# seiya-kumada/3d_gaussian_splatting

Measured on AMD Instinct MI355X. Metric: forward+backward iters/s at 1080p, 1M Gaussians; PSNR vs CPU ref, higher is better.
Workload: dtype f32; 1 GPU; 1m_1080p: 1000000 Gaussians, 1920x1080, SH degree 3, fwd+bwd; gaussians=1000000, width=1920, height=1080, sh_degree=3, parallelism=single GPU

## Files before the change

### 3d_gaussian_splatting_amd/csrc/gsr_blend.hip

```cpp
#include "gsr_kernels.h"

namespace gsr {
namespace {

constexpr int kPPL = 4;

__device__ inline int xcd_tile(int b, int nwg) {
    const int q = nwg / 8, r = nwg % 8;
    const int xcd = b % 8, local = b / 8;
    return (xcd < r ? xcd * (q + 1) : r * (q + 1) + (xcd - r) * q) + local;
}

template <int CTRL>
__device__ inline float dpp_f(float x) {
    return __int_as_float(__builtin_amdgcn_update_dpp(0, __float_as_int(x), CTRL, 0xF, 0xF, false));
}

template <int N>
__device__ __forceinline__ void quad_reduce(float (&v)[N]) {
#pragma unroll
    for (int i = 0; i < N; ++i) v[i] += dpp_f<0xB1>(v[i]);
#pragma unroll
    for (int i = 0; i < N; ++i) v[i] += dpp_f<0x4E>(v[i]);
#pragma unroll
    for (int i = 0; i < N; ++i) asm volatile("" : "+v"(v[i]));
}



struct BlendGeom {
    int W, H, grid_x, ty0, nwg;
    int vgy, vh;
    uint32_t ck_slots;
    int ck_fixed;
    float bg0, bg1, bg2;
    uint32_t cap;
};

__device__ __forceinline__ float edge_min_q(float a, float b, float c, float k, float u, float v0, float v1) {
    const float vs = fminf(fmaxf(k * u, v0), v1);
    return fmaf(fmaf(c, vs, b * u), vs, a * u * u);
}

__device__ inline uint32_t stripe_mask(const float4 r0, const float4 r1, const float4 r2, float bx0, float by0) {
    const float ex = r2.y, ey = r2.z;
    if (!(ex >= 0.0f) || r0.x + ex < bx0 || r0.x - ex > bx0 + 15.0f) return 0u;
    const float ylo = r0.y - ey, yhi = r0.y + ey;
    const float A = -r0.z, B = -r0.w, C = -r1.x;
    const bool pd = A > 0.0f && C > 0.0f && 4.0f * A * C - B * B > 0.0f;
    const float bound = fmaf(fmaxf(r2.w + 7.99435343f, 0.0f), 1.02f, 0.05f);
    const float x0 = bx0 - r0.x, x1 = bx0 + 15.0f - r0.x;
    const float kc = -B * __builtin_amdgcn_rcpf(2.0f * C), ka = -B * __builtin_amdgcn_rcpf(2.0f * A);
    uint32_t m = 0;
#pragma unroll
    for (int p = 0; p < kPPL; ++p) {
        const float s0 = by0 + 4.0f * p;
        bool hit = yhi >= s0 && ylo <= s0 + 3.0f;
        if (hit && pd) {
            const float y0 = s0 - r0.y, y1 = s0 + 3.0f - r0.y;
            const bool inside = x0 <= 0.0f && x1 >= 0.0f && y0 <= 0.0f && y1 >= 0.0f;
            const float q = fminf(fminf(edge_min_q(A, B, C, kc, x0, y0, y1), edge_min_q(A, B, C, kc, x1, y0, y1)),
                                  fminf(edge_min_q(C, B, A, ka, y0, x0, x1), edge_min_q(C, B, A, ka, y1, x0, x1)));
            hit = inside || q <= bound;
        }
        m |= hit ? (1u << p) : 0u;
    }
    return m;
}

__device__ __forceinline__ float pair_alpha(float e, float L, float& oG) {
    oG = __builtin_amdgcn_exp2f(e);
    const float a = __builtin_amdgcn_fmed3f(oG, 0.0f, 0.99f);
    return (e <= L && oG >= (1.0f / 255.0f)) ? a : 0.0f;
}

__device__ __forceinline__ float pair_alpha_keep(float e, float L, float& oG, bool& keep) {
    oG = __builtin_amdgcn_exp2f(e);
    keep = e <= L && oG >= (1.0f / 255.0f);
    return keep ? __builtin_amdgcn_fmed3f(oG, 0.0f, 0.99f) : 0.0f;
}


constexpr int kF6Batch4 = 256;
constexpr int kF6Wpe = 8;
template <class T>
__device__ __forceinline__ T aux_arg() { return T{}; }
template <class T>
__device__ __forceinline__ T aux_arg(const T& a) { return a; }
__device__ __forceinline__ float aux_value(uint32_t key, int inv) {
    const float z = __uint_as_float(key);
    return inv ? 1.0f / z : z;
}
constexpr int kF6AuxWpe = 7;
template <int NW, class... AX>
__global__ __launch_bounds__(64 * NW) __attribute__((amdgpu_waves_per_eu(NW == 2 ? (sizeof...(AX) ? kF6AuxWpe : kF6Wpe) : 1))) void blend_forward_kernel(const BlendGeom geo,
                                                                const uint2* __restrict__ ranges,
                                                                const uint32_t* __restrict__ sorted_gid,
                                                                const float4* __restrict__ rec,
                                                                float* __restrict__ out_color,
                                                                float* __restrict__ final_T,
                                                                float* __restrict__ accum,
                                                                uint32_t* __restrict__ term,
                                                                float4* __restrict__ ck,
                                                                uint8_t* __restrict__ mk, const AX... axp) {
    constexpr bool AUX = sizeof...(AX) > 0;
    static_assert(sizeof...(AX) <= 1, "one aux argument");
    const F6Aux ax = aux_arg<F6Aux>(axp...);
    constexpr int PPL = kPPL / NW;
    constexpr int BATCH = NW > 2 ? kF6Batch4 : 64 * NW;
    static_assert(BATCH % 64 == 0 && BATCH <= 64 * NW, "F6 batch");
    constexpr int kCW = NW > 2 ? kBandChunkWork : kChunkWork;
    __shared__ float4 srec[BATCH * 3];
    __shared__ uint32_t smk[BATCH];
    __shared__ uint32_t slive[NW];
    __shared__ float svz[AUX ? BATCH : 1];
    const int tl = xcd_tile(blockIdx.x, geo.nwg);
    const int tile = tl + geo.ty0 * geo.grid_x;
    const int tx = tile % geo.grid_x, ty = tile / geo.grid_x;
    const int tid = threadIdx.x, w = tid >> 6, lane = tid & 63;
    const int px = tx * kTile + (lane & 15);
    const float pfx = (float)px;
    const int view = ty / geo.vgy, tyl = ty - view * geo.vgy;
    const float bx0 = (float)(tx * kTile), by0 = (float)(tyl * kTile);
    float pfy[PPL], T[PPL], C0[PPL], C1[PPL], C2[PPL];
    float Z[PPL];
#pragma unroll
    for (int p = 0; p < PPL; ++p) {
        const int pyl = tyl * kTile + (lane >> 4) + 4 * (w * PPL + p);
        pfy[p] = (float)pyl;
        T[p] = (px < geo.W && pyl < geo.vh) ? 1.0f : -1.0f;
        C0[p] = C1[p] = C2[p] = 0.0f;
        Z[p] = 0.0f;
    }
    const uint2 range = ranges[tile];
    const int n = (int)(range.y - range.x);
    float vref = 0.0f;
    if constexpr (AUX) {
        if (n > 0) vref = aux_value(ax.depth_key[sorted_gid[range.x]], ax.inv);
    }
    uint32_t* const table = term + (size_t)tl * kMaxChunks;
    int nck = 0;
    int work = 0;
    int tend = n;
    uint8_t* const ckm = reinterpret_cast<uint8_t*>(ck + (size_t)geo.ck_slots * 256);
    auto checkpoint = [&](size_t slot, uint32_t lv) {
        float4* dst = ck + (size_t)slot * 256;
#pragma unroll
        for (int p = 0; p < PPL; ++p) {
            const bool on = (lv >> p) & 1u;
            if (on) dst[64 * (w * PPL + p) + lane] = make_float4(T[p], C0[p], C1[p], C2[p]);
            if constexpr (AUX) {
                if (on) ax.ckz[(size_t)slot * 256 + 64 * (w * PPL + p) + lane] = Z[p];
            }
            if (lane == 0) ckm[4 * (size_t)slot + w * PPL + p] = on ? 1 : 0;
        }
    };
    int quota = kCW;
    auto merge_chunks = [&]() {
        constexpr int kKeep = (kMaxChunks - 1) / 2;
        float4* const ckt = ck + ck_slot_of(geo.ck_fixed, range.x, tl, 1) * 256 - 256;
        uint8_t* const ckmt = ckm + (ck_slot_of(geo.ck_fixed, range.x, tl, 1) - 1) * 4;
#pragma unroll 1
        for (int k = 1; k <= kKeep; ++k) {
#pragma unroll 1
            for (int p = 0; p < PPL; ++p) {
                const int i = 64 * (w * PPL + p) + lane;
                ckt[256 * k + i] = ckt[512 * k + i];
                if constexpr (AUX) {
                    float* const ckzt = ax.ckz + ck_slot_of(geo.ck_fixed, range.x, tl, 1) * 256 - 256;
                    ckzt[256 * k + i] = ckzt[512 * k + i];
                }
                if (lane == 0) ckmt[4 * k + w * PPL + p] = ckmt[8 * k + w * PPL + p];
            }
            if (tid == 0) table[k] = table[2 * k];
        }
        nck = kKeep;
        work += quota;
        quota *= 2;
    };
    uint32_t g_next = tid < BATCH && tid < n ? sorted_gid[range.x + tid] : 0u;
    for (int base = 0; base < n; base += BATCH) {
        uint32_t live = 0;
#pragma unroll
        for (int p = 0; p < PPL; ++p) live |= __any(T[p] > 0.0f) ? (1u << p) : 0u;
        if (lane == 0) slive[w] = live << (w * PPL);
        if (tid < BATCH && base + tid < n) {
            const uint32_t g = g_next;
            if (base + BATCH + tid < n) g_next = sorted_gid[range.x + base + BATCH + tid];
            const float4* r = rec + 3 * (size_t)g;
            const float4 r0 = r[0], r1 = r[1], r2 = r[2];
            srec[3 * tid + 0] = r0;
            srec[3 * tid + 1] = r1;
            srec[3 * tid + 2] = r2;
            smk[tid] = stripe_mask(r0, r1, r2, bx0, by0);
            if constexpr (AUX) svz[tid] = aux_value(ax.depth_key[g], ax.inv) - vref;
            mk[range.x + base + tid] = (uint8_t)smk[tid];
        } else if (tid < BATCH) {
            smk[tid] = 0u;
        }
        __syncthreads();
        uint32_t tile_live = 0;
#pragma unroll
        for (int i = 0; i < NW; ++i) tile_live |= slive[i];
        if (tile_live == 0) {
            tend = base;
            break;
        }
        const int cnt = (n - base) < BATCH ? (n - base) : BATCH;
        int visited = 0;
        for (int c0 = 0; c0 < cnt; c0 += 64) {
            const uint32_t sm = smk[c0 + lane];
            if (__builtin_expect(work >= quota && nck == kMaxChunks - 1, 0)) merge_chunks();
            if (work >= quota && nck < kMaxChunks - 1) {
                ++nck;
                checkpoint(ck_slot_of(geo.ck_fixed, range.x, tl, nck), live);
                if (tid == 0) table[nck] = (uint32_t)(base + c0);
                work = 0;
            }
            const uint32_t tm = sm & tile_live;
            work += __popcll(__ballot(tm & 1u)) + __popcll(__ballot(tm & 2u)) + __popcll(__ballot(tm & 4u)) +
                    __popcll(__ballot(tm & 8u));
            if (!live) continue;
            const uint32_t mine = (sm >> (w * PPL)) & ((1u << PPL) - 1u);
            uint64_t todo = __ballot((mine & live) != 0u && c0 + lane < cnt);
            if constexpr (PPL == 1) {
                while (todo) {
                    const int ka = c0 + __builtin_ctzll(todo);
                    todo &= todo - 1;
                    const bool two = todo != 0;
                    const int kb = two ? c0 + __builtin_ctzll(todo) : ka;
                    if (two) todo &= todo - 1;
                    const float4 a0 = srec[3 * ka + 0], a1 = srec[3 * ka + 1], a2 = srec[3 * ka + 2];
                    const float4 b0 = srec[3 * kb + 0], b1 = srec[3 * kb + 1], b2 = srec[3 * kb + 2];
                    const float dxa = a0.x - pfx, dxb = b0.x - pfx;
                    const float dya = a0.y - pfy[0], dyb = b0.y - pfy[0];
                    const float ea = fmaf(fmaf(a1.x, dya, a0.w * dxa), dya, fmaf(a0.z * dxa, dxa, a2.w));
                    const float eb = fmaf(fmaf(b1.x, dyb, b0.w * dxb), dyb, fmaf(b0.z * dxb, dxb, b2.w));
                    float oGa, oGb;
                    const float aa = pair_alpha(ea, a2.w, oGa);
                    const float ab = pair_alpha(eb, b2.w, oGb);
                    {
                        const float w = aa * T[0];
                        const float tT = T[0] - w;
                        const bool ok = tT >= 0.0001f;
                        const float wgt = ok ? w : 0.0f;
                        C0[0] = fmaf(a1.z, wgt, C0[0]);
                        C1[0] = fmaf(a1.w, wgt, C1[0]);
                        C2[0] = fmaf(a2.x, wgt, C2[0]);
                        if constexpr (AUX) Z[0] = fmaf(svz[ka], wgt, Z[0]);
                        T[0] = ok ? tT : -fabsf(T[0]);
                    }
                    if (two) {
                        const float w = ab * T[0];
                        const float tT = T[0] - w;
                        const bool ok = tT >= 0.0001f;
                        const float wgt = ok ? w : 0.0f;
                        C0[0] = fmaf(b1.z, wgt, C0[0]);
                        C1[0] = fmaf(b1.w, wgt, C1[0]);
                        C2[0] = fmaf(b2.x, wgt, C2[0]);
                        if constexpr (AUX) Z[0] = fmaf(svz[kb], wgt, Z[0]);
                        T[0] = ok ? tT : -fabsf(T[0]);
                    }
                    const int before = visited;
                    visited += two ? 2 : 1;
                    if ((before >> 3) != (visited >> 3)) {
                        live = __any(T[0] > 0.0f) ? 1u : 0u;
                        if (live == 0) break;
                    }
                }
                continue;
            }
            while (todo) {
                const int kk = __builtin_ctzll(todo);
                todo &= todo - 1;
                const int k = c0 + kk;
                const float4 r0 = srec[3 * k + 0];
                const float4 r1 = srec[3 * k + 1];
                const float4 r2 = srec[3 * k + 2];
                const float dx = r0.x - pfx;
                const float bdx = r0.w * dx;
                const float K = fmaf(r0.z * dx, dx, r2.w);
                float vz = 0.0f;
                if constexpr (AUX) vz = svz[k];
#pragma unroll
                for (int p = 0; p < PPL; ++p) {
                    const float dy = r0.y - pfy[p];
                    const float e = fmaf(fmaf(r1.x, dy, bdx), dy, K);
                    float oG;
                    const float a = pair_alpha(e, r2.w, oG);
                    const float w = a * T[p];
                    const float tT = T[p] - w;
                    const bool ok = tT >= 0.0001f;
                    const float wgt = ok ? w : 0.0f;
                    C0[p] = fmaf(r1.z, wgt, C0[p]);
                    C1[p] = fmaf(r1.w, wgt, C1[p]);
                    C2[p] = fmaf(r2.x, wgt, C2[p]);
                    if constexpr (AUX) Z[p] = fmaf(vz, wgt, Z[p]);
                    T[p] = ok ? tT : -fabsf(T[p]);
                }
                if ((++visited & 7) == 0) {
                    uint32_t lv = 0;
#pragma unroll
                    for (int p = 0; p < PPL; ++p) lv |= __any(T[p] > 0.0f) ? (1u << p) : 0u;
                    live = lv;
                    if (live == 0) break;
                }
            }
        }
        __syncthreads();
    }
    if (tid == 0) {
        table[0] = (uint32_t)tend;
        for (int c = nck + 1; c < kMaxChunks; ++c) table[c] = 0xFFFFFFFFu;
    }
    const size_t npix = (size_t)geo.W * geo.vh;
    float* const oc = out_color + (size_t)view * 3 * npix;
    float* const ac = accum + (size_t)view * 3 * npix;
    float* const fT = final_T + (size_t)view * npix;
#pragma unroll
    for (int p = 0; p < PPL; ++p) {
        const int pyl = tyl * kTile + (lane >> 4) + 4 * (w * PPL + p);
        if (px < geo.W && pyl < geo.vh) {
            const size_t pix = (size_t)pyl * geo.W + px;
            const float Tf = fabsf(T[p]);
            fT[pix] = Tf;
            ac[pix] = C0[p];
            ac[npix + pix] = C1[p];
            ac[2 * npix + pix] = C2[p];
            oc[pix] = C0[p] + Tf * geo.bg0;
            oc[npix + pix] = C1[p] + Tf * geo.bg1;
            oc[2 * npix + pix] = C2[p] + Tf * geo.bg2;
            if constexpr (AUX) {
                ax.accum_z[pix] = Z[p];
                ax.out_depth[pix] = fmaf(vref, 1.0f - Tf, Z[p]);
                ax.out_alpha[pix] = 1.0f - Tf;
            }
        }
    }
}

constexpr int kPark = 4;
constexpr int kParkSlot = 16 * 12 + 8;
static_assert(kParkSlot % 32 == 8 && kParkSlot % 4 == 0, "flush banks / float4 alignment");
template <bool AUX = false>
__device__ __forceinline__ void park_flush(const float* qpark, const uint32_t* sjl, uint32_t kpack, int parked,
                                           float* p8f, float* p1, uint8_t* fl, int lane, float* pz = nullptr) {
    __syncthreads();
    const int slot = lane & 3, c = lane >> 2;
    if (c < (AUX ? 10 : 9) && slot < parked) {
        const float* q = qpark + slot * kParkSlot + c;
        float t[4] = {-0.f, -0.f, -0.f, -0.f};
#pragma unroll
        for (int i = 0; i < 16; ++i) t[i & 3] += q[i * 12];
        const uint32_t j = sjl[(kpack >> (6 * slot)) & 63u];
        if (j != 0xFFFFFFFFu) {
            float* dst = c < 8 ? p8f + 8 * (size_t)j + c : p1 + j;
            if constexpr (AUX) dst = c == 9 ? pz + j : dst;
            *dst = (t[0] + t[1]) + (t[2] + t[3]);
            if (c == 8) fl[j] = 1;
        }
    }
    __syncthreads();
}

constexpr int kB1AuxWpe = 5;
template <bool PF = false, class... AX>
__global__ __launch_bounds__(64) __attribute__((amdgpu_waves_per_eu(PF ? 4 : (sizeof...(AX) ? kB1AuxWpe : 6)))) void blend_backward_kernel(const BlendGeom geo,
                                                            const uint2* __restrict__ ranges,
                                                            const uint32_t* __restrict__ sorted_gid,
                                                            const uint4* __restrict__ rect,
                                                            const float4* __restrict__ rec,
                                                            const float* __restrict__ final_T,
                                                            const float* __restrict__ accum,
                                                            const float* __restrict__ dL_dpix,
                                                            float* __restrict__ p8f,
                                                            float* __restrict__ p1,
                                                            uint8_t* __restrict__ fl,
                                                            const uint32_t* __restrict__ term,
                                                            const float4* __restrict__ ck,
                                                            const uint8_t* __restrict__ mk, const AX... axp) {
    constexpr bool AUX = sizeof...(AX) > 0;
    static_assert(sizeof...(AX) <= 1, "one aux argument");
    constexpr int SPW = kPPL;
    const B1Aux ax = aux_arg<B1Aux>(axp...);
    __shared__ float svz[AUX ? 64 : 1];
    __shared__ struct {
        float4 srec[64 * 3];
        uint32_t sjl[64];
        float qpark[kPark * kParkSlot];
        uint32_t sidx[64];
        uint32_t smv[64];
        uint32_t sgd[64];
    } lds;
    float4* const srec = lds.srec;
    uint32_t* const sjl = lds.sjl;
    float* const qpark = lds.qpark;
    const int lane = threadIdx.x;
    float* const qlane = qpark + (lane >> 2) * 12;
    int tl, chunk;
    {
        const int q = geo.nwg / 8, r = geo.nwg % 8, xcd = blockIdx.x % 8, local = (int)(blockIdx.x / 8);
        const int t0 = xcd < r ? xcd * (q + 1) : r * (q + 1) + (xcd - r) * q, nt = q + (xcd < r ? 1 : 0);
        const int per = q + 1;
        chunk = local / per;
        const int i = local - chunk * per;
        if (i >= nt) return;
        tl = t0 + i;
    }
    const int tile = tl + geo.ty0 * geo.grid_x;
    const uint2 range = ranges[tile];
    const int n_all = (int)(range.y - range.x);
    const uint32_t* table = term + (size_t)tl * kMaxChunks;
    const uint32_t tend = table[0];
    const uint32_t start_u = chunk == 0 ? 0u : table[chunk];
    if (start_u >= (uint32_t)n_all || start_u >= tend) return;
    const int start = (int)start_u;
    float vref = 0.0f;
    if constexpr (AUX) vref = aux_value(ax.depth_key[sorted_gid[range.x]], ax.inv);
    const uint32_t next = chunk + 1 < kMaxChunks ? table[chunk + 1] : 0xFFFFFFFFu;
    const int n = next < (uint32_t)n_all ? (int)next : n_all;
    const int tx = tile % geo.grid_x, ty = tile / geo.grid_x;
    const int col = lane >> 2, row = lane & 3;
    const int px = tx * kTile + col;
    const float pfx = (float)px;
    const int view = ty / geo.vgy, tyl = ty - view * geo.vgy;
    const size_t npix = (size_t)geo.W * geo.vh;
    final_T += (size_t)view * npix;
    accum += (size_t)view * 3 * npix;
    dL_dpix += (size_t)view * 3 * npix;
    float pfy[SPW], T[SPW], R[SPW], dp0[SPW], dp1[SPW], dp2[SPW];
    float dpz[SPW], v0[SPW], azS[SPW], azT[SPW], azA[SPW];
#pragma unroll
    for (int p = 0; p < SPW; ++p) {
        const int pyl = tyl * kTile + row + 4 * p;
        pfy[p] = (float)pyl;
        const bool in = px < geo.W && pyl < geo.vh;
        const size_t pix = in ? (size_t)pyl * geo.W + px : 0;
        const float Tfin = in ? final_T[pix] : 1.0f;
        dp0[p] = in ? dL_dpix[pix] : 0.0f;
        dp1[p] = in ? dL_dpix[npix + pix] : 0.0f;
        dp2[p] = in ? dL_dpix[2 * npix + pix] : 0.0f;
        const float sdp = in ? accum[pix] * dp0[p] + accum[npix + pix] * dp1[p] + accum[2 * npix + pix] * dp2[p]
                             : 0.0f;
        R[p] = sdp + Tfin * (geo.bg0 * dp0[p] + geo.bg1 * dp1[p] + geo.bg2 * dp2[p]);
        dpz[p] = 0.0f;
        if constexpr (AUX) {
            dpz[p] = in && ax.dL_ddepth ? ax.dL_ddepth[pix] : 0.0f;
            azA[p] = in && ax.dL_dalpha ? ax.dL_dalpha[pix] : 0.0f;
            azS[p] = in ? ax.accum_z[pix] : 0.0f;
            azT[p] = Tfin;
            const float atot = 1.0f - Tfin;
            v0[p] = atot > 1e-6f ? azS[p] / atot : 0.0f;
        } else {
            v0[p] = azS[p] = azT[p] = azA[p] = 0.0f;
        }
        T[p] = in ? 1.0f : -1.0f;
    }
    if (chunk > 0) {
        const size_t slot = ck_slot_of(geo.ck_fixed, range.x, tl, chunk);
        const float4* src = ck + slot * 256;
        const uint32_t on = *reinterpret_cast<const uint32_t*>(
            reinterpret_cast<const uint8_t*>(ck + (size_t)geo.ck_slots * 256) + 4 * slot);
#pragma unroll
        for (int p = 0; p < SPW; ++p) {
            if ((on >> (8 * p)) & 0xFFu) {
                const float4 c4 = src[64 * p + col + 16 * row];
                T[p] = c4.x;
                R[p] -= fmaf(c4.y, dp0[p], fmaf(c4.z, dp1[p], c4.w * dp2[p]));
                if constexpr (AUX) azS[p] -= ax.ckz[slot * 256 + 64 * p + col + 16 * row];
            } else {
                T[p] = -1.0f;
            }
        }
    }
    if constexpr (AUX) {
#pragma unroll
        for (int p = 0; p < SPW; ++p) {
            const float Tst = chunk > 0 ? fabsf(T[p]) : 1.0f;
            const float rem = azS[p] - v0[p] * (Tst - azT[p]);
            R[p] = R[p] + ((rem - (v0[p] + vref) * azT[p]) * dpz[p] - azT[p] * azA[p]);
        }
    }
    const int n_lim = n < (int)tend ? n : (int)tend;
    for (int base = start; base < n_lim;) {
        uint32_t live = 0;
#pragma unroll
        for (int p = 0; p < SPW; ++p) live |= __any(T[p] > 0.0f) ? (1u << p) : 0u;
        if (live == 0) break;
        static_assert(kB1Win == 4, "one mask word and four gids per lane");
        const uint32_t a0 = (range.x + (uint32_t)base) & ~(uint32_t)(kB1Win - 1);
        const uint32_t wd = *reinterpret_cast<const uint32_t*>(mk + a0 + 4 * lane);
        const uint4 gw = *reinterpret_cast<const uint4*>(sorted_gid + a0 + 4 * lane);
        const uint32_t gwa[4] = {gw.x, gw.y, gw.z, gw.w};
        uint32_t vis = 0;
#pragma unroll
        for (int i = 0; i < kB1Win; ++i) {
            const int e = (int)(a0 + kB1Win * lane + i - range.x);
            const uint32_t m = (wd >> (8 * i)) & 0xFu;
            if (e >= base && e < n_lim && (m & live)) vis |= 1u << i;
        }
        const uint32_t c = (uint32_t)__popc(vis);
        uint32_t incl = c;
#pragma unroll
        for (int o = 1; o < 64; o <<= 1) {
            const uint32_t y = __shfl_up(incl, o, 64);
            if (lane >= o) incl += y;
        }
        const uint32_t excl = incl - c;
        const uint32_t total = (uint32_t)__shfl(incl, 63, 64);
        const int cnt = total < 64u ? (int)total : 64;
        uint32_t pos = excl;
#pragma unroll
        for (int i = 0; i < kB1Win; ++i) {
            if ((vis >> i) & 1u) {
                if (pos < 64u) {
                    lds.sidx[pos] = a0 + kB1Win * lane + i - range.x;
                    lds.smv[pos] = (wd >> (8 * i)) & 0xFu;
                    lds.sgd[pos] = gwa[i];
                }
                ++pos;
            }
        }
        __syncthreads();
        base = total > 64u ? (int)lds.sidx[63] + 1 : (int)(a0 + 64 * kB1Win - range.x);
        if (cnt == 0) {
            __syncthreads();
            continue;
        }
        uint32_t jl = 0, smask = 0;
        if (lane < cnt) {
            const uint32_t g = lds.sgd[lane];
            const uint4 rr = rect[g];
            const int minx = rr.x & 0xFFFF, miny = rr.x >> 16, maxx = rr.y & 0xFFFF;
            const int y0 = miny > geo.ty0 ? miny : geo.ty0;
            jl = rr.z + (uint32_t)((ty - y0) * (maxx - minx) + (tx - minx));
            if (jl >= geo.cap) jl = 0xFFFFFFFFu;
            const float4* r = rec + 3 * (size_t)g;
            srec[3 * lane + 0] = r[0];
            srec[3 * lane + 1] = r[1];
            srec[3 * lane + 2] = r[2];
            if constexpr (AUX) svz[lane] = aux_value(ax.depth_key[g], ax.inv) - vref;
            smask = lds.smv[lane];
        }
        sjl[lane] = jl;
        __syncthreads();
        uint64_t todo = __ballot(lane < cnt);
        int visited = 0, parked = 0;
        uint32_t kpack = 0;
        auto record = [&](const int k, const float4 r0, const float4 r1, const float4 r2, const float vz) -> bool {
            const uint32_t m = (uint32_t)__builtin_amdgcn_readlane((int)smask, k) & live;
            const float dx = r0.x - pfx;
            const float bdx = r0.w * dx;
            const float K = fmaf(r0.z * dx, dx, r2.w);
            float s0 = -0.f, sy = -0.f, syy = -0.f, g0 = -0.f, g1 = -0.f, g2 = -0.f;
            float gz = -0.f;
            bool any = false;
            auto contribute = [&](const int p, const float a, const float w, const float oG, const float dy) {
                any = true;
                const float one_m = 1.0f - a;
                float cdp = fmaf(r1.z, dp0[p], fmaf(r1.w, dp1[p], r2.x * dp2[p]));
                if constexpr (AUX) {
                    cdp = fmaf(vz - v0[p], dpz[p], cdp);
                    gz = fmaf(w, dpz[p], gz);
                }
                R[p] = fmaf(-w, cdp, R[p]);
                const float dLda = fmaf(T[p], cdp, -R[p] * __builtin_amdgcn_rcpf(one_m));
                g0 = fmaf(w, dp0[p], g0);
                g1 = fmaf(w, dp1[p], g1);
                g2 = fmaf(w, dp2[p], g2);
                const float sv = oG * dLda;
                s0 += sv;
                const float svy = sv * dy;
                sy += svy;
                syy = fmaf(svy, dy, syy);
            };
#pragma unroll
            for (int p = 0; p < SPW; ++p) {
                if (!(m & (1u << p))) continue;
                const float dy = r0.y - pfy[p];
                const float e = fmaf(fmaf(r1.x, dy, bdx), dy, K);
                float oG;
                bool keep;
                const float a = pair_alpha_keep(e, r2.w, oG, keep);
                const float w = a * T[p];
                const float tT = T[p] - w;
                const bool ok = tT >= 0.0001f;
                if (ok && keep) contribute(p, a, w, oG, dy);
                T[p] = ok ? tT : -fabsf(T[p]);
            }
            if (__any(any)) {
                float u[AUX ? 7 : 6] = {s0, sy, syy, g0, g1, g2};
                if constexpr (AUX) u[6] = gz;
                quad_reduce(u);
                const float sx = u[0] * dx;
                float v[9] = {sx, u[1], sx * dx, u[1] * dx, u[2], u[0], u[3], u[4], u[5]};
                if ((lane & 3) == 0) {
                    float* dst = qlane + parked * kParkSlot;
                    *reinterpret_cast<float4*>(dst) = make_float4(v[0], v[1], v[2], v[3]);
                    *reinterpret_cast<float4*>(dst + 4) = make_float4(v[4], v[5], v[6], v[7]);
                    dst[8] = v[8];
                    if constexpr (AUX) dst[9] = u[6];
                }
                kpack |= (uint32_t)k << (6 * parked);
                if (++parked == kPark) {
                    park_flush<AUX>(qpark, sjl, kpack, parked, p8f, p1, fl, lane, ax.pz);
                    parked = 0;
                    kpack = 0;
                }
            }
            if ((++visited & 7) == 0) {
                uint32_t lv = 0;
#pragma unroll
                for (int p = 0; p < SPW; ++p) lv |= __any(T[p] > 0.0f) ? (1u << p) : 0u;
                live = lv;
                if (live == 0) return true;
            }
            return false;
        };
        if constexpr (PF) {
            if (todo) {
                int ka = __builtin_ctzll(todo);
                todo &= todo - 1;
                float4 a0 = srec[3 * ka + 0], a1 = srec[3 * ka + 1], a2 = srec[3 * ka + 2];
                float4 b0, b1, b2;
                float za = 0.0f, zb = 0.0f;
                if constexpr (AUX) za = svz[ka];
                while (true) {
                    const int kb = todo ? __builtin_ctzll(todo) : -1;
                    if (kb >= 0) {
                        todo &= todo - 1;
                        b0 = srec[3 * kb + 0];
                        b1 = srec[3 * kb + 1];
                        b2 = srec[3 * kb + 2];
                        if constexpr (AUX) zb = svz[kb];
                    }
                    if (record(ka, a0, a1, a2, za) || kb < 0) break;
                    ka = todo ? __builtin_ctzll(todo) : -1;
                    if (ka >= 0) {
                        todo &= todo - 1;
                        a0 = srec[3 * ka + 0];
                        a1 = srec[3 * ka + 1];
                        a2 = srec[3 * ka + 2];
                        if constexpr (AUX) za = svz[ka];
                    }
                    if (record(kb, b0, b1, b2, zb) || ka < 0) break;
                }
            }
        } else {
            while (todo) {
                const int k = __builtin_ctzll(todo);
                todo &= todo - 1;
                float vz = 0.0f;
                if constexpr (AUX) vz = svz[k];
                if (record(k, srec[3 * k + 0], srec[3 * k + 1], srec[3 * k + 2], vz)) break;
            }
        }
        if (parked) park_flush<AUX>(qpark, sjl, kpack, parked, p8f, p1, fl, lane, ax.pz);
        __syncthreads();
    }
}
}

constexpr int kF6FullWaves = 2, kF6BandWaves = 4, kF6BandTiles = 4096;

static BlendGeom make_geo(const gsr_camera& cam, const float bg[3], int ty0, int ty1, long long cap, int vgy, int vh) {
    BlendGeom g;
    g.W = cam.width;
    g.H = cam.height;
    g.vgy = vgy > 0 ? vgy : div_up(cam.height, kTile);
    g.vh = vgy > 0 ? vh : cam.height;
    g.grid_x = div_up(cam.width, kTile);
    g.ty0 = ty0;
    g.nwg = (ty1 - ty0) * g.grid_x;
    const long long full_tiles = (long long)div_up(cam.height, kTile) * g.grid_x;
    g.ck_slots = (uint32_t)ck_pool_slots(cap, full_tiles);
    g.ck_fixed = ck_fixed_layout(cap, full_tiles) ? 1 : 0;
    g.bg0 = bg[0];
    g.bg1 = bg[1];
    g.bg2 = bg[2];
    g.cap = cap > 0 ? (uint32_t)cap : 0u;
    return g;
}

static long long image_tiles(const BlendGeom& geo, int vgy) {
    return vgy > 0 ? (long long)geo.vgy * geo.grid_x : geo.nwg;
}
static bool aux_ok(const void* aux, const gsr_camera& cam, int ty0, int ty1, int vgy) {
    return !aux || (vgy <= 0 && ty0 == 0 && ty1 == div_up(cam.height, kTile));
}

int launch_blend_forward(const gsr_camera& cam, const float bg[3], int ty0, int ty1,
                         const uint2* ranges, const uint32_t* sorted_gid, const float4* rec,
                         float* out_color, float* final_T, float* accum, uint32_t* term, float4* ck, long long cap,
                         hipStream_t s, int vgy, int vh, uint8_t* mk, const F6Aux* aux) {
    if (!aux_ok(aux, cam, ty0, ty1, vgy)) return (int)hipErrorInvalidValue;
    const BlendGeom geo = make_geo(cam, bg, ty0, ty1, cap, vgy, vh);
    if (geo.nwg <= 0) return 0;
    auto launch = [&](auto nw, auto... ax) {
        constexpr int NW = decltype(nw)::value;
        hipLaunchKernelGGL((blend_forward_kernel<NW, decltype(ax)...>), dim3(geo.nwg), dim3(64 * NW), 0, s, geo, ranges,
                           sorted_gid, rec, out_color, final_T, accum, term, ck, mk, ax...);
    };
    auto pick = [&](auto... ax) {
        if (image_tiles(geo, vgy) >= kF6BandTiles)
            launch(std::integral_constant<int, kF6FullWaves>{}, ax...);
        else
            launch(std::integral_constant<int, kF6BandWaves>{}, ax...);
    };
    aux ? pick(*aux) : pick();
    return (int)hipGetLastError();
}

int launch_blend_backward(const gsr_camera& cam, const float bg[3], int ty0, int ty1,
                          const uint2* ranges, const uint32_t* sorted_gid, const uint4* rect,
                          const float4* rec, const float* final_T,
                          const float* accum, const float* dL_dpix, float* partial, long long cap,
                          const uint32_t* term, const float4* ck, hipStream_t s, int vgy, int vh,
                          const uint8_t* mk, const B1Aux* aux) {
    if (!aux_ok(aux, cam, ty0, ty1, vgy)) return (int)hipErrorInvalidValue;
    const BlendGeom geo = make_geo(cam, bg, ty0, ty1, cap, vgy, vh);
    if (geo.nwg <= 0) return 0;
    const PartLayout pl(cap, aux != nullptr);
    const int blocks = 8 * (geo.nwg / 8 + 1) * kMaxChunks;
    auto launch = [&](auto pf, auto... ax) {
        hipLaunchKernelGGL((blend_backward_kernel<decltype(pf)::value, decltype(ax)...>), dim3(blocks), dim3(64), 0, s,
                           geo, ranges, sorted_gid, rect, rec, final_T, accum, dL_dpix, at<float>(partial, pl.p8),
                           at<float>(partial, pl.p1), at<uint8_t>(partial, pl.fl), term, ck, mk, ax...);
    };
    auto pick = [&](auto... ax) {
        if (image_tiles(geo, vgy) < kF6BandTiles)
            launch(std::true_type{}, ax...);
        else
            launch(std::false_type{}, ax...);
    };
    B1Aux ax = aux ? *aux : B1Aux{};
    ax.pz = at<float>(partial, pl.pz);
    aux ? pick(ax) : pick();
    return (int)hipGetLastError();
}

int launch_clear_flags(float* partial, long long cap, bool aux, hipStream_t s) {
    if (cap <= 0) return 0;
    return (int)hipMemsetAsync(at<uint8_t>(partial, PartLayout(cap, aux).fl), 0, (size_t)cap, s);
}

}
```

Measured before the change: 923.7 iters/s.

## Compact staged Gaussian records in LDS and make park flushes bank-conflict-free

```diff
diff --git a/3d_gaussian_splatting_amd/csrc/gsr_blend.hip b/3d_gaussian_splatting_amd/csrc/gsr_blend.hip
--- a/3d_gaussian_splatting_amd/csrc/gsr_blend.hip
+++ b/3d_gaussian_splatting_amd/csrc/gsr_blend.hip
@@ -319,7 +319,7 @@
     float* const fT = final_T + (size_t)view * npix;
 #pragma unroll
     for (int p = 0; p < PPL; ++p) {
-        const int pyl = tyl * kTile + (lane >> 4) + 4 * (w * PPL + p);
+        const int pyl = (int)pfy[p];
         if (px < geo.W && pyl < geo.vh) {
             const size_t pix = (size_t)pyl * geo.W + px;
             const float Tf = fabsf(T[p]);
@@ -339,25 +339,76 @@
     }
 }
 
+constexpr int kStagedRec = 10;
+struct StagedRec {
+    float4 r0;
+    float4 h;
+    float L;
+};
+__device__ __forceinline__ StagedRec staged(const float2* srec, int k) {
+    const float2* p = srec + k * (kStagedRec / 2);
+    const float2 a = p[0], b = p[1], c = p[2], d = p[3];
+    return {make_float4(a.x, a.y, b.x, b.y), make_float4(c.x, c.y, d.x, d.y), p[4].x};
+}
+
 constexpr int kPark = 4;
-constexpr int kParkSlot = 16 * 12 + 8;
-static_assert(kParkSlot % 32 == 8 && kParkSlot % 4 == 0, "flush banks / float4 alignment");
+constexpr int kParkSlot = 16 * 12 + (kPark <= 4 ? 8 : 12);
+static_assert(kPark <= 5 && kParkSlot % 4 == 0, "flush banks / float4 alignment of the leaders' stores");
+struct FlushMap {
+    uint8_t sc[64];
+    bool ok;
+};
+constexpr FlushMap make_flush_map(int moments) {
+    FlushMap m{};
+    for (int l = 0; l < 64; ++l) m.sc[l] = 0xFF;
+    m.ok = true;
+    bool used[2][32] = {};
+    int fill[2] = {0, 0};
+    for (int s = 0; s < kPark; ++s)
+        for (int c = 0; c < moments; ++c) {
+            const int bank = (s * kParkSlot + c) % 32;
+            const int g = used[0][bank] ? 1 : 0;
+            if (used[g][bank] || fill[g] == 32) {
+                m.ok = false;
+                continue;
+            }
+            used[g][bank] = true;
+            m.sc[32 * g + fill[g]++] = (uint8_t)(s << 4 | c);
+        }
+    return m;
+}
+__device__ constexpr FlushMap kFlushMap = make_flush_map(9), kFlushMapAux = make_flush_map(10);
+static_assert(kFlushMap.ok && kFlushMapAux.ok, "flush lanes of one group on one LDS bank");
+static_assert(6 * kPark <= 32, "kpack");
+typedef const __attribute__((address_space(3))) float* LdsFloats;
+struct FlushLane {
+    LdsFloats q;
+    char* base;
+    uint32_t step;
+    int slot;
+    bool flag;
+};
 template <bool AUX = false>
-__device__ __forceinline__ void park_flush(const float* qpark, const uint32_t* sjl, uint32_t kpack, int parked,
-                                           float* p8f, float* p1, uint8_t* fl, int lane, float* pz = nullptr) {
+__device__ __forceinline__ FlushLane flush_lane(int lane, const float* qpark, float* p8f, float* p1, float* pz) {
+    const int sc = AUX ? kFlushMapAux.sc[lane] : kFlushMap.sc[lane];
+    const int c = sc & 15, slot = sc == 0xFF ? kPark : sc >> 4;
+    float* b = c < 8 ? p8f + c : p1;
+    if constexpr (AUX) b = c == 9 ? pz : b;
+    LdsFloats q = (LdsFloats)(qpark + (sc == 0xFF ? 0 : slot * kParkSlot + c));
+    asm volatile("" : "+v"(q));
+    return {q, reinterpret_cast<char*>(b), c < 8 ? 32u : 4u, slot, c == 8};
+}
+__device__ __forceinline__ void park_flush(const FlushLane f, const float2* srec, uint32_t kpack, int parked,
+                                           uint8_t* fl) {
     __syncthreads();
-    const int slot = lane & 3, c = lane >> 2;
-    if (c < (AUX ? 10 : 9) && slot < parked) {
-        const float* q = qpark + slot * kParkSlot + c;
+    if (f.slot < parked) {
         float t[4] = {-0.f, -0.f, -0.f, -0.f};
 #pragma unroll
-        for (int i = 0; i < 16; ++i) t[i & 3] += q[i * 12];
-        const uint32_t j = sjl[(kpack >> (6 * slot)) & 63u];
+        for (int i = 0; i < 16; ++i) t[i & 3] += f.q[i * 12];
+        const uint32_t j = __float_as_uint(srec[((kpack >> (6 * f.slot)) & 63u) * (kStagedRec / 2) + 4].y);
         if (j != 0xFFFFFFFFu) {
-            float* dst = c < 8 ? p8f + 8 * (size_t)j + c : p1 + j;
-            if constexpr (AUX) dst = c == 9 ? pz + j : dst;
-            *dst = (t[0] + t[1]) + (t[2] + t[3]);
-            if (c == 8) fl[j] = 1;
+            *reinterpret_cast<float*>(f.base + (size_t)j * f.step) = (t[0] + t[1]) + (t[2] + t[3]);
+            if (f.flag) fl[j] = 1;
         }
     }
     __syncthreads();
@@ -385,15 +436,17 @@
     const B1Aux ax = aux_arg<B1Aux>(axp...);
     __shared__ float svz[AUX ? 64 : 1];
     __shared__ struct {
-        float4 srec[64 * 3];
-        uint32_t sjl[64];
-        float qpark[kPark * kParkSlot];
-        uint32_t sidx[64];
-        uint32_t smv[64];
-        uint32_t sgd[64];
+        float2 srec[64 * kStagedRec / 2];
+        union {
+            float qpark[kPark * kParkSlot];
+            struct {
+                uint32_t sidx[64];
+                uint32_t smv[64];
+                uint32_t sgd[64];
+            };
+        };
     } lds;
-    float4* const srec = lds.srec;
-    uint32_t* const sjl = lds.sjl;
+    float2* const srec = lds.srec;
     float* const qpark = lds.qpark;
     const int lane = threadIdx.x;
     float* const qlane = qpark + (lane >> 2) * 12;
@@ -482,6 +535,7 @@
         }
     }
     const int n_lim = n < (int)tend ? n : (int)tend;
+    const FlushLane flane = flush_lane<AUX>(lane, qpark, p8f, p1, ax.pz);
     for (int base = start; base < n_lim;) {
         uint32_t live = 0;
 #pragma unroll
@@ -536,27 +590,30 @@
             jl = rr.z + (uint32_t)((ty - y0) * (maxx - minx) + (tx - minx));
             if (jl >= geo.cap) jl = 0xFFFFFFFFu;
             const float4* r = rec + 3 * (size_t)g;
-            srec[3 * lane + 0] = r[0];
-            srec[3 * lane + 1] = r[1];
-            srec[3 * lane + 2] = r[2];
+            const float4 r0 = r[0], r1 = r[1], r2 = r[2];
+            float2* const d = srec + lane * (kStagedRec / 2);
+            d[0] = make_float2(r0.x, r0.y);
+            d[1] = make_float2(r0.z, r0.w);
+            d[2] = make_float2(r1.x, r1.z);
+            d[3] = make_float2(r1.w, r2.x);
+            d[4] = make_float2(r2.w, __uint_as_float(jl));
             if constexpr (AUX) svz[lane] = aux_value(ax.depth_key[g], ax.inv) - vref;
             smask = lds.smv[lane];
         }
-        sjl[lane] = jl;
         __syncthreads();
         uint64_t todo = __ballot(lane < cnt);
         int visited = 0, parked = 0;
         uint32_t kpack = 0;
-        auto record = [&](const int k, const float4 r0, const float4 r1, const float4 r2, const float vz) -> bool {
+        auto record = [&](const int k, const StagedRec sr, const float vz) -> bool {
+            const float4 r0 = sr.r0, r1 = make_float4(sr.h.x, 0.0f, sr.h.y, sr.h.z), r2 = make_float4(sr.h.w, 0.0f, 0.0f, sr.L);
             const uint32_t m = (uint32_t)__builtin_amdgcn_readlane((int)smask, k) & live;
             const float dx = r0.x - pfx;
             const float bdx = r0.w * dx;
             const float K = fmaf(r0.z * dx, dx, r2.w);
             float s0 = -0.f, sy = -0.f, syy = -0.f, g0 = -0.f, g1 = -0.f, g2 = -0.f;
             float gz = -0.f;
-            bool any = false;
+            uint64_t any = 0;
             auto contribute = [&](const int p, const float a, const float w, const float oG, const float dy) {
-                any = true;
                 const float one_m = 1.0f - a;
                 float cdp = fmaf(r1.z, dp0[p], fmaf(r1.w, dp1[p], r2.x * dp2[p]));
                 if constexpr (AUX) {
@@ -585,10 +642,12 @@
                 const float w = a * T[p];
                 const float tT = T[p] - w;
                 const bool ok = tT >= 0.0001f;
+                any |= __builtin_amdgcn_fcmpf(tT, 0.0001f, 3) & __builtin_amdgcn_fcmpf(e, r2.w, 5) &
+                       __builtin_amdgcn_fcmpf(oG, 1.0f / 255.0f, 3);
                 if (ok && keep) contribute(p, a, w, oG, dy);
                 T[p] = ok ? tT : -fabsf(T[p]);
             }
-            if (__any(any)) {
+            if (any) {
                 float u[AUX ? 7 : 6] = {s0, sy, syy, g0, g1, g2};
                 if constexpr (AUX) u[6] = gz;
                 quad_reduce(u);
@@ -603,7 +662,7 @@
                 }
                 kpack |= (uint32_t)k << (6 * parked);
                 if (++parked == kPark) {
-                    park_flush<AUX>(qpark, sjl, kpack, parked, p8f, p1, fl, lane, ax.pz);
+                    park_flush(flane, srec, kpack, kPark, fl);
                     parked = 0;
                     kpack = 0;
                 }
@@ -621,29 +680,24 @@
             if (todo) {
                 int ka = __builtin_ctzll(todo);
                 todo &= todo - 1;
-                float4 a0 = srec[3 * ka + 0], a1 = srec[3 * ka + 1], a2 = srec[3 * ka + 2];
-                float4 b0, b1, b2;
+                StagedRec ra = staged(srec, ka), rb;
                 float za = 0.0f, zb = 0.0f;
                 if constexpr (AUX) za = svz[ka];
                 while (true) {
                     const int kb = todo ? __builtin_ctzll(todo) : -1;
                     if (kb >= 0) {
                         todo &= todo - 1;
-                        b0 = srec[3 * kb + 0];
-                        b1 = srec[3 * kb + 1];
-                        b2 = srec[3 * kb + 2];
+                        rb = staged(srec, kb);
                         if constexpr (AUX) zb = svz[kb];
                     }
-                    if (record(ka, a0, a1, a2, za) || kb < 0) break;
+                    if (record(ka, ra, za) || kb < 0) break;
                     ka = todo ? __builtin_ctzll(todo) : -1;
                     if (ka >= 0) {
                         todo &= todo - 1;
-                        a0 = srec[3 * ka + 0];
-                        a1 = srec[3 * ka + 1];
-                        a2 = srec[3 * ka + 2];
+                        ra = staged(srec, ka);
                         if constexpr (AUX) za = svz[ka];
                     }
-                    if (record(kb, b0, b1, b2, zb) || ka < 0) break;
+                    if (record(kb, rb, zb) || ka < 0) break;
                 }
             }
         } else {
@@ -652,10 +706,10 @@
                 todo &= todo - 1;
                 float vz = 0.0f;
                 if constexpr (AUX) vz = svz[k];
-                if (record(k, srec[3 * k + 0], srec[3 * k + 1], srec[3 * k + 2], vz)) break;
-            }
-        }
-        if (parked) park_flush<AUX>(qpark, sjl, kpack, parked, p8f, p1, fl, lane, ax.pz);
+                if (record(k, staged(srec, k), vz)) break;
+            }
+        }
+        if (parked) park_flush(flane, srec, kpack, parked, fl);
         __syncthreads();
     }
 }
```

Measured after the change: 949.2 iters/s, median of 6. 2.8% higher.
